# talmolab/VNL-Brax-Imitation

Measured on AMD Instinct MI355X. Metric: env-steps/sec (whole node), rodent imitation, num_envs=4096/GPU, higher is better.
Workload: dtype f32; 1 GPU; rodent imitation rollout, single groom clip, 4096 envs/GPU: intention-policy forward (HIP) -> RodentTracking.step (5 substeps, CG 6/6) -> auto-reset on -> Transition logging (unroll 20, the 20 steps replayed as one captured hipGraph); envs_per_gpu=4096, clips=1, parallelism=env-sharded x1, no data-path collective

## Files before the change

__graft_entry__.py:

```python
from __future__ import annotations

import os
import sys

ROOT = os.path.dirname(os.path.abspath(__file__))
if ROOT not in sys.path:
    sys.path.insert(0, ROOT)


def build() -> None:
    import vnl_brax_imitation_amd
    from vnl_brax_imitation_amd.csrc import build as hip_build

    from concurrent.futures import ThreadPoolExecutor

    with ThreadPoolExecutor(7) as pool:
        futs = {v: pool.submit(hip_build.build, variant=v)
                for v in ("product", "spill", "noblk", "nospec", "tail", "plain", "vmemplain")}
        paths = {v: f.result() for v, f in futs.items()}
    path = paths["product"]
    assert all(os.path.exists(p_) for p_ in paths.values()), paths
    from oracle import oracle as _oracle

    _oracle.build()
    from vnl_brax_imitation_amd import _lib

    _lib.load_library(path)
    print(f"[build] {path} ok; oracle ok")


def smoke() -> None:
    import numpy as np
    import torch

    sys.path.insert(0, os.path.join(ROOT, "tests"))
    import helpers as H
    from vnl_brax_imitation_amd.envs.rodent import RodentTracking

    assert torch.cuda.is_available(), "smoke() needs a HIP device"
    B = 256
    env = RodentTracking(H.reference_clip(), num_envs=B, device="cuda:0", **H.env_kwargs())
    rng = np.random.default_rng(0)
    sf = rng.integers(0, 235, B).astype(np.int32)
    noise = (1e-3 * rng.standard_normal((B, 74))).astype(np.float32)
    st = env.reset(start_frame=torch.from_numpy(sf), noise=torch.from_numpy(noise))
    act = np.clip(0.3 * rng.standard_normal((B, 30)), -1, 1).astype(np.float32)
    o = H.make_oracle(env, "f64")
    ost = o.env_reset(sf, noise)
    e_reset = H.scaled_err(st.pipeline_state.qacc_warmstart.cpu().numpy(), ost["qacc_warmstart"])
    e_obs = H.scaled_err(st.obs.cpu().numpy(), ost["obs"])
    import parity as P

    o32 = H.make_oracle(env, "f32")
    st, err, dev, rep, ost = P.control_step_follow(env, o, o32, sf, noise, act)
    torch.cuda.synchronize()
    print(f"[smoke] reset qacc err {e_reset:.2e}, obs err {e_obs:.2e}; control step vs oracle (following the product's "
          f"solver decisions): qvel err max {err['qvel'].max():.2e} median {np.median(err['qvel']):.2e}, qpos max "
          f"{err['qpos'].max():.2e}; reward {st.reward.mean().item():.5f} vs {ost['reward'].mean():.5f}")
    w = int(np.argmax(err["qvel"]))
    print(f"[smoke] worst env {w}: product vs float64 oracle {err['qvel'][w]:.2e}, float32 oracle vs float64 oracle "
          f"{dev['qvel'][w]:.2e} on the same env (bound: max(1e-5, {P.K_SENS} x that))")
    cp, co = P.compliance(err), P.compliance(dev)
    print(f"[smoke] envs within 1e-5 after ONE CONTROL STEP ({B} envs): product qpos {cp['qpos']:.3f} qvel {cp['qvel']:.3f} | "
          f"float32 oracle qpos {co['qpos']:.3f} qvel {co['qvel']:.3f}")
    env1 = RodentTracking(H.reference_clip(), num_envs=B, device="cuda:0", **{**H.env_kwargs(), "n_frames": 1})
    o1, o1_32 = H.make_oracle(env1, "f64"), H.make_oracle(env1, "f32")
    _, err1, dev1, rep1, _ = P.control_step_follow(env1, o1, o1_32, sf, noise, act)
    cp1, co1 = P.compliance(err1), P.compliance(dev1)
    print(f"[smoke] envs within 1e-5 after ONE SUBSTEP: product qpos {cp1['qpos']:.3f} qvel {cp1['qvel']:.3f} | float32 oracle "
          f"qpos {co1['qpos']:.3f} qvel {co1['qvel']:.3f}; followed decisions: {P.assert_legitimate(rep1)}")
    for f, idx in P.bound_violations(err1, dev1).items():
# ... 13 lines not shown
```

vnl-brax-imitation_amd/csrc/build.py:

```python
from __future__ import annotations

import os
import subprocess
import sys

HERE = os.path.dirname(os.path.abspath(__file__))
SOURCES = ["vnl_lib.hip", "vnl_policy.hip", "vnl_ppo.hip", "vnl_domain.hip"]
DEPS = SOURCES + ["vnl_env_kernels.h", "vnl_body.h", "vnl_types.h", "vnl_philox.h", "vnl_policy_train.h", "../../include/vnl.h"]
OUT = os.path.join(HERE, "libvnl.so")

VARIANTS = {
    "product": ("libvnl.so", ["-DVNL_KERNEL_ATTR=__attribute__((amdgpu_waves_per_eu(2,2)))"]),
    "prof": ("libvnl_prof.so", ["-DVNL_PROFILE", "-DVNL_KERNEL_ATTR=__attribute__((amdgpu_waves_per_eu(2,2)))"]),
    "knobs": ("libvnl_knobs.so", ["-DVNL_STAGE_KNOBS", "-DVNL_KERNEL_ATTR=__attribute__((amdgpu_waves_per_eu(2,2)))"]),
    "spill": ("libvnl_spill.so", ["-DVNL_KERNEL_ATTR=__attribute__((amdgpu_waves_per_eu(4,4)))"]),
    "noblk": ("libvnl_noblk.so", ["-DVNL_NO_BLK", "-DVNL_KERNEL_ATTR=__attribute__((amdgpu_waves_per_eu(2,2)))"]),
    "tail": ("libvnl_tail.so", ["-DVNL_SOLVER_TAIL", "-DVNL_KERNEL_ATTR=__attribute__((amdgpu_waves_per_eu(2,2)))"]),
    "plain": ("libvnl_plain.so", ["-DVNL_SOLVER_PLAIN", "-DVNL_KERNEL_ATTR=__attribute__((amdgpu_waves_per_eu(2,2)))"]),
    "vmemplain": ("libvnl_vmemplain.so", ["-DVNL_VMEM_PLAIN", "-DVNL_KERNEL_ATTR=__attribute__((amdgpu_waves_per_eu(2,2)))"]),
    "nospec": ("libvnl_nospec.so", ["-DVNL_NO_SPEC", "-DVNL_KERNEL_ATTR=__attribute__((amdgpu_waves_per_eu(2,2)))"]),
}
ENV_KERNELS = ("vnl_step_kernel", "vnl_reset_kernel", "vnl_reset_done_kernel")


def resource_usage(stderr_text: str) -> dict:
    out, name = {}, None
    for line in stderr_text.splitlines():
        if "Function Name:" in line:
            name = line.split("Function Name:")[1].split()[0]
            out[name] = {}
        elif name and "remark:" in line:
            body = line.split("remark:")[1].split("[-Rpass")[0].strip()
            key, _, val = body.rpartition(":")
            try:
                out[name][key.strip()] = int(val.strip())
            except ValueError:
                pass
    return out


def build(force: bool = False, verbose: bool = False, profile: bool = False, knobs: bool = False,
          variant: str | None = None) -> str:
    variant = variant or ("prof" if profile else ("knobs" if knobs else "product"))
    fname, defs = VARIANTS[variant]
    out = os.path.join(HERE, fname)
    deps = [os.path.join(HERE, d) for d in DEPS] + [os.path.abspath(__file__)]
    newest = max(os.path.getmtime(d) for d in deps)
    if not force and os.path.exists(out) and os.path.getmtime(out) >= newest:
        return out
    hipcc = os.environ.get("HIPCC", "/opt/rocm/bin/hipcc")
    objdir = os.path.join(HERE, "_obj", variant)
    os.makedirs(objdir, exist_ok=True)
    flags = ["-Rpass-analysis=kernel-resource-usage", "--offload-arch=gfx950", "-O3", "-fno-slp-vectorize", "-std=c++17", "-fPIC"] + \
        defs + os.environ.get("VNL_HIPCC_EXTRA", "").split()
    stamp = " ".join(flags)
    headers = [d for d in deps if not d.endswith(".hip")]
    SRC_DEPS = {"vnl_lib.hip": headers, "vnl_policy.hip": [h for h in headers if h.endswith("vnl.h")] + [os.path.join(HERE, "vnl_policy_train.h"), os.path.join(HERE, "vnl_philox.h")],
                "vnl_ppo.hip": [h for h in headers if h.endswith("vnl.h")] + [os.path.join(HERE, "vnl_policy_train.h")]}
    objs, remarks = [], ""
    for src in SOURCES:
        obj = os.path.join(objdir, src + ".o")
        rem = obj + ".remarks.txt"
        srcdeps = [os.path.join(HERE, src)] + [h for h in SRC_DEPS.get(src, headers) if os.path.exists(h)]
        fresh = (not force and os.path.exists(obj) and os.path.exists(rem) and
                 os.path.getmtime(obj) >= max(os.path.getmtime(d) for d in srcdeps) and
                 open(rem).readline().rstrip("\n") == stamp)
        if not fresh:
            cmd = [hipcc] + flags + ["-c", os.path.join(HERE, src), "-o", obj]
            if verbose:
                print(" ".join(cmd), file=sys.stderr)
            r = subprocess.run(cmd, stderr=subprocess.PIPE, text=True)
            if verbose or r.returncode:
# ... 48 lines not shown
```

vnl-brax-imitation_amd/csrc/vnl_body.h:

```cpp
#pragma once
#include <math.h>

#include "vnl_types.h"

#ifndef VNL_HD
#define VNL_HD __device__ __forceinline__
#endif
#include "vnl_philox.h"

#ifndef VNL_FORKJOIN_DEFINED
#define VNL_LANES 64
#define VNL_ROWS_PER_LANE 8
#define VNL_ROWS_SMALL 5
#define VNL_CHAIN_WIDTH 8
#define VNL_ROWSETS_1 1
#define VNL_ROWSETS_2 2
#define VNL_FOR(i, n) for (int i = (int)lane; i < (n); i += VNL_LANES)
#define VNL_SERIAL if (lane == 0)
#define VNL_SYNC() __builtin_amdgcn_fence(__ATOMIC_ACQ_REL, "wavefront")
#define VNL_SYNC_GLOBAL()                                     \
  do {                                                        \
    __builtin_amdgcn_fence(__ATOMIC_ACQ_REL, "wavefront");    \
    asm volatile("s_waitcnt vmcnt(0)" ::: "memory");          \
    __builtin_amdgcn_fence(__ATOMIC_ACQ_REL, "wavefront");    \
  } while (0)
#define VNL_LDS_DECL(name) extern __shared__ __align__(16) vreal name[]
VNL_HD float vnl_wave_sum(float x) {
#define VNL_DPP_STEP(ctrl) x += __builtin_bit_cast(float, __builtin_amdgcn_update_dpp(0, __builtin_bit_cast(int, x), ctrl, 0xf, 0xf, true))
  VNL_DPP_STEP(0xB1);
  VNL_DPP_STEP(0x4E);
  VNL_DPP_STEP(0x141);
  VNL_DPP_STEP(0x140);
#undef VNL_DPP_STEP
  x += __builtin_bit_cast(float, __builtin_amdgcn_update_dpp(0, __builtin_bit_cast(int, x), 0x142, 0xa, 0xf, false));
  x += __builtin_bit_cast(float, __builtin_amdgcn_update_dpp(0, __builtin_bit_cast(int, x), 0x143, 0xc, 0xf, false));
  return __builtin_bit_cast(float, __builtin_amdgcn_readlane(__builtin_bit_cast(int, x), 63));
}
VNL_HD float vnl_wave_sum16(float x) {
#define VNL_DPP_STEP(ctrl) x += __builtin_bit_cast(float, __builtin_amdgcn_update_dpp(0, __builtin_bit_cast(int, x), ctrl, 0xf, 0xf, true))
  VNL_DPP_STEP(0xB1);
  VNL_DPP_STEP(0x4E);
  VNL_DPP_STEP(0x141);
  VNL_DPP_STEP(0x140);
#undef VNL_DPP_STEP
  return __builtin_bit_cast(float, __builtin_amdgcn_readlane(__builtin_bit_cast(int, x), 0));
}
VNL_HD bool vnl_wave_any(bool x) { return __ballot(x) != 0ull; }
VNL_HD float vnl_wave_scan(float x) {
#define VNL_DPP_SCAN(ctrl, rmask) \
  x += __builtin_bit_cast(float, __builtin_amdgcn_update_dpp(0, __builtin_bit_cast(int, x), ctrl, rmask, 0xf, false))
  VNL_DPP_SCAN(0x111, 0xf);
  VNL_DPP_SCAN(0x112, 0xf);
  VNL_DPP_SCAN(0x114, 0xf);
  VNL_DPP_SCAN(0x118, 0xf);
// ... 84 lines not shown
}
VNL_HD V3 qrot(V3 v, Q4 q) {
  V3 u = v3(q.x, q.y, q.z);
  vreal uv = dot(u, v), uu = dot(u, u);
  V3 c = cross(u, v);
  return u * (vreal(2.) * uv) + v * (q.w * q.w - uu) + c * (vreal(2.) * q.w);
}
struct M3 {
  vreal a[9];
};
VNL_HD M3 qmat(Q4 q) {
  M3 m;
  vreal q00 = q.w * q.w, q01 = q.w * q.x, q02 = q.w * q.y, q03 = q.w * q.z;
  vreal q11 = q.x * q.x, q12 = q.x * q.y, q13 = q.x * q.z, q22 = q.y * q.y, q23 = q.y * q.z, q33 = q.z * q.z;
  m.a[0] = q00 + q11 - q22 - q33, m.a[1] = vreal(2.) * (q12 - q03), m.a[2] = vreal(2.) * (q13 + q02);
  m.a[3] = vreal(2.) * (q12 + q03), m.a[4] = q00 - q11 + q22 - q33, m.a[5] = vreal(2.) * (q23 - q01);
  m.a[6] = vreal(2.) * (q13 - q02), m.a[7] = vreal(2.) * (q23 + q01), m.a[8] = q00 - q11 - q22 + q33;
  return m;
}
VNL_HD V3 mmul(const M3& m, V3 v) {
  return V3{m.a[0] * v.x + m.a[1] * v.y + m.a[2] * v.z, m.a[3] * v.x + m.a[4] * v.y + m.a[5] * v.z,
            m.a[6] * v.x + m.a[7] * v.y + m.a[8] * v.z};
}
struct S6 {
  V3 a, l;
};
VNL_HD S6 operator+(S6 p, S6 q) { return S6{p.a + q.a, p.l + q.l}; }
VNL_HD S6 operator*(S6 p, vreal s) { return S6{p.a * s, p.l * s}; }
VNL_HD vreal dot(S6 p, S6 q) { return dot(p.a, q.a) + dot(p.l, q.l); }
VNL_HD S6 mcross(S6 u, S6 v) { return S6{cross(u.a, v.a), cross(u.l, v.a) + cross(u.a, v.l)}; }
VNL_HD S6 mcross_force(S6 v, S6 f) { return S6{cross(v.a, f.a) + cross(v.l, f.l), cross(v.a, f.l)}; }

#if defined(__HIP_DEVICE_COMPILE__)
#define VNL_CAS __attribute__((address_space(4)))
#define VNL_TO_CAS(T, p) ((const VNL_CAS T*)(unsigned long long)(p))
#define VNL_LAUNDER(p) asm volatile("" : "+s"(p))
#else
#define VNL_CAS
#define VNL_TO_CAS(T, p) ((const T*)(p))
#define VNL_LAUNDER(p)
#endif
#define MI(f) (SP::fixed ? SP::D.f : m.f)
#define LO(f) (SP::fixed ? SP::L.f : L.f)
#if defined(__HIP_DEVICE_COMPILE__)
#define VNL_GLOBAL_PTR(T, p) ((const __attribute__((address_space(1))) T*)(p))
#else
#define VNL_GLOBAL_PTR(T, p) ((const T*)(p))
#endif
#if defined(__HIP_DEVICE_COMPILE__) && !defined(VNL_VMEM_PLAIN)
#define VNL_PIN(x) asm volatile("" : "+v"(x))
#else
#define VNL_PIN(x) (void)(x)
#endif
#if defined(__HIP_DEVICE_COMPILE__) && !defined(VNL_SOLVER_PLAIN)
#define VNL_SOLVE_REGS 1
#else
#define VNL_SOLVE_REGS 0
#endif
#define VNL_BLK_REGS 2
#define VNL_LIMROW_REGS 2
#define VNL_SR_BLK 1
#define VNL_SR_LIMROW 2
struct VnlSolveRegs {
  int on;
  unsigned blk[2][VNL_BLK_REGS];
  int limrow[VNL_LIMROW_REGS];
};
template <class SP>
struct EnvWaveT {
  const VNL_CAS DevModel& m;
  const VNL_CAS DevEnv& ev;
  const DevState& st;
  const VNL_CAS WsLayout& L;
  vreal* s;
  unsigned e, lane;
  const VNL_CAS KernelConsts* kc;
  int* trace;
  VnlSolveRegs sr;
  VNL_HD EnvWaveT with_trace(int* t) const { return EnvWaveT{m, ev, st, L, s, e, lane, kc, t, sr}; }
  VNL_HD EnvWaveT fresh() const {
    const VNL_CAS KernelConsts* k = kc;
    VNL_LAUNDER(k);
    return EnvWaveT{k->m, k->ev, st, k->L, s, e, lane, k, trace, sr};
  }
  VNL_HD EnvWaveT with_solve_regs(bool with_limrow) const {
    EnvWaveT w = *this;
#if VNL_SOLVE_REGS
    const int cfg = MI(blk_cfg), tr = cfg & 15, tc = (cfg >> 4) & 15;
    const bool blk = blk_on();
#pragma unroll
    for (int t = 0; t < VNL_BLK_REGS; t++) {
      w.sr.blk[0][t] = (blk && t < tr) ? m.blk_tab[t * 64 + (int)lane] : 0u;
      w.sr.blk[1][t] = (blk && t < tc) ? m.blk_tab[(tr + t) * 64 + (int)lane] : 0u;
    }
#pragma unroll
    for (int q = 0; q < VNL_LIMROW_REGS; q++) {
      const int d = (int)lane + 64 * q;
      w.sr.limrow[q] = (with_limrow && d < MI(nv)) ? m.dof_limrow[d] : 0;
    }
#pragma unroll
    for (int t = 0; t < VNL_BLK_REGS; t++) asm volatile("" : "+v"(w.sr.blk[0][t]), "+v"(w.sr.blk[1][t]));
    if (with_limrow) {
#pragma unroll
      for (int q = 0; q < VNL_LIMROW_REGS; q++) asm volatile("" : "+v"(w.sr.limrow[q]));
    }
    w.sr.on = with_limrow ? (VNL_SR_BLK | VNL_SR_LIMROW) : VNL_SR_BLK;
// ... 654 lines not shown
        if (u < qd(q)) pb[u] = s + LDb + (u < d ? madr(anc_of(adr + u)) : 0);
#pragma unroll
      for (int t = 1; t < MAXD; t++) {
        if (t < qd(q) && vnl_wave_any(t <= d)) {
          vreal x[MAXD];
#pragma unroll
          for (int u = 1; u < t; u++) x[u] = pb[u][t - u];
          vreal acc = t <= d ? -s[own + t] : vreal(0.);
#pragma unroll
          for (int u = 1; u < t; u++) acc -= nn[u] * x[u];
          nn[t] = acc;
        }
      }
      VNL_SYNC();
#pragma unroll
      for (int t = 1; t < MAXD; t++)
        if (t < qd(q) && t <= d) s[own + t] = nn[t];
      VNL_SYNC();
    }
  }

  template <int NSET>
  VNL_HD void factor_aba(vreal h) const {
    constexpr int LW = 16;
    const int sc = (LO(Mgrad) + 3) & ~3;
    const int VS = vstore();
    vreal* g2 = fac2();
    const int nsteps = MI(fac_steps);
    v2r U[NSET][6], diag[NSET];
    vreal S[NSET][6];
    int dep[NSET], ftime[NSET], myline[NSET], adrs[NSET];
#ifdef VNL_VMEM_PLAIN
    const unsigned char* mt[NSET];
    unsigned nxt[NSET];
#else
    constexpr int NW = SP::fixed ? vnl_imax(vnl_fac_stride(SP::D.fac_steps) / 4, 1) : 4;
    const int nwords = vnl_fac_stride(nsteps) / 4;
    const auto* mw = VNL_GLOBAL_PTR(unsigned, m.fac_match);
    unsigned woff[NSET], win[NSET][NW], wcur[NSET];
    auto pick_word = [&](int q, int i) {
      unsigned r = win[q][0];
#pragma unroll
      for (int k = 1; k < NW; k++) {
        unsigned w = win[q][k];
        VNL_PIN(w);
        r = i == k ? w : r;
      }
      return r;
    };
    auto load_window = [&](int q, bool ok, int w0) {
#pragma unroll
      for (int i = 0; i < NW; i++) win[q][i] = (ok && w0 + i < nwords) ? mw[woff[q] + (unsigned)(w0 + i)] : 0u;
    };
    vreal inv2[NSET];
#endif
#pragma unroll
    for (int q = 0; q < NSET; q++) {
      const int a = (int)lane + q * VNL_LANES;
      const bool ok = a < MI(nv);
      const int aa = ok ? a : 0;
      const S6 c = ld6(LO(cdof) + 6 * aa), f = inert_mul(LO(P) + 10 * m.dof_body[aa], c);
      S[q][0] = c.a.x, S[q][1] = c.a.y, S[q][2] = c.a.z, S[q][3] = c.l.x, S[q][4] = c.l.y, S[q][5] = c.l.z;
      U[q][0] = v2r{f.a.x, f.a.x}, U[q][1] = v2r{f.a.y, f.a.y}, U[q][2] = v2r{f.a.z, f.a.z};
      U[q][3] = v2r{f.l.x, f.l.x}, U[q][4] = v2r{f.l.y, f.l.y}, U[q][5] = v2r{f.l.z, f.l.z};
      const vreal arm = par<P_ARM>(aa);
      diag[q] = v2r{arm, arm + h * par<P_DAMP>(aa)};
      adrs[q] = madr(aa), dep[q] = eadr(aa) - adrs[q];
      myline[q] = m.dof_fslot[aa];
      ftime[q] = ok ? m.dof_ftime[aa] : -1;
#ifdef VNL_VMEM_PLAIN
      mt[q] = m.fac_match + (size_t)aa * vnl_fac_stride(nsteps);
      nxt[q] = (ok && nsteps > 0) ? mt[q][0] : 0u;
#else
      woff[q] = (unsigned)(aa * nwords);
      load_window(q, ok, 0);
      wcur[q] = win[q][0];
      inv2[q] = vreal(0.);
#endif
    }
    VNL_SYNC();
    VNL_PROF(7);
    for (int step = 0; step < nsteps; step++) {
      unsigned cur[NSET];
#pragma unroll
      for (int q = 0; q < NSET; q++) {
#ifdef VNL_VMEM_PLAIN
        cur[q] = nxt[q];
        nxt[q] = (ftime[q] >= 0 && step + 1 < nsteps) ? mt[q][step + 1] : 0u;
#else
        cur[q] = wcur[q] & 0xffu, wcur[q] >>= 8;
#endif
        if (ftime[q] == step) {
          const int a = (int)lane + q * VNL_LANES;
          v2r D = diag[q];
#pragma unroll
          for (int i = 0; i < 6; i++) D += v2r{S[q][i], S[q][i]} * U[q][i];
          const v2r iv = v2r{vnl_recip(D[0]), vnl_recip(D[1])};
          vreal* ln = s + sc + myline[q] * LW;
          st4a(ln, U[q][0][0], U[q][0][1], U[q][1][0], U[q][1][1]);
          st4a(ln + 4, U[q][2][0], U[q][2][1], U[q][3][0], U[q][3][1]);
          st4a(ln + 8, U[q][4][0], U[q][4][1], U[q][5][0], U[q][5][1]);
          st4a(ln + 12, iv[0], iv[1], (vreal)(adrs[q] + dep[q]), vreal(0.));
          vreal* vs = s + VS + 12 * a;
          const v2r v0 = U[q][0] * iv, v1 = U[q][1] * iv, v2 = U[q][2] * iv, v3_ = U[q][3] * iv, v4 = U[q][4] * iv, v5 = U[q][5] * iv;
          st4a(vs, v0[0], v0[1], v1[0], v1[1]);
          st4a(vs + 4, v2[0], v2[1], v3_[0], v3_[1]);
          st4a(vs + 8, v4[0], v4[1], v5[0], v5[1]);
          s[LO(dinv) + a] = iv[0];
#ifdef VNL_VMEM_PLAIN
          g2[MI(nM) + a] = iv[1];
#else
          inv2[q] = iv[1];
#endif
        }
      }
      VNL_WAVE_FENCE();
      for (int pass = 0; pass < VNL_FAC_LINES; pass++) {
        bool more = false;
#pragma unroll
        for (int q = 0; q < NSET; q++) more = more || cur[q] != 0u;
        if (!vnl_wave_any(more)) break;
#pragma unroll
        for (int q = 0; q < NSET; q++) {
          if (cur[q] != 0u) {
            const int k = __builtin_ctz(cur[q]);
            cur[q] &= cur[q] - 1u;
            const vreal* ln = s + sc + k * LW;
            const R4 u0 = ld4a(ln), u1 = ld4a(ln + 4), u2 = ld4a(ln + 8), hd = ld4a(ln + 12);
            const v2r Uk[6] = {v2r{u0.x, u0.y}, v2r{u0.z, u0.w}, v2r{u1.x, u1.y}, v2r{u1.z, u1.w}, v2r{u2.x, u2.y}, v2r{u2.z, u2.w}};
            v2r pa = v2r{S[q][0], S[q][0]} * Uk[0], pb = v2r{S[q][1], S[q][1]} * Uk[1];
            pa += v2r{S[q][2], S[q][2]} * Uk[2], pb += v2r{S[q][3], S[q][3]} * Uk[3];
            pa += v2r{S[q][4], S[q][4]} * Uk[4], pb += v2r{S[q][5], S[q][5]} * Uk[5];
            const v2r Lk = (pa + pb) * v2r{hd.x, hd.y};
#pragma unroll
            for (int i = 0; i < 6; i++) U[q][i] -= Lk * Uk[i];
            s[LO(LD) + (int)hd.z - dep[q]] = Lk[0];
          }
        }
      }
      VNL_WAVE_FENCE();
#ifndef VNL_VMEM_PLAIN
      if ((step & 3) == 3) {
        const int wi = (step >> 2) + 1;
#pragma unroll
        for (int q = 0; q < NSET; q++) {
          if (!SP::fixed && wi % NW == 0) load_window(q, ftime[q] >= 0, wi);
          wcur[q] = pick_word(q, wi % NW);
        }
      }
#endif
    }
#ifndef VNL_VMEM_PLAIN
#pragma unroll
    for (int q = 0; q < NSET; q++)
      if (ftime[q] >= 0) g2[MI(nM) + (int)lane + q * VNL_LANES] = inv2[q];
#endif
    VNL_SYNC();
    VNL_PROF(8);
    VNL_PROF(9);
  }

  VNL_HD int vstore() const { return vnl_vstore(LO(P)); }
  VNL_HD int cvel_at() const { return vnl_cvel_at(LO(P), LO(smooth), MI(nbody), MI(nv)); }

  template <int NSET, bool GUESTS>
  VNL_HD void invert_aba(vreal* g2) const {
    const int VS = vstore();
    const unsigned char* an = (const unsigned char*)(s + LO(tab_anc));
    auto load_v = [&](int r, v2r* C) {
      const vreal* vs = s + VS + 12 * r;
      const R4 a = ld4a(vs), b = ld4a(vs + 4), c = ld4a(vs + 8);
      C[0] = v2r{a.x, a.y}, C[1] = v2r{a.z, a.w}, C[2] = v2r{b.x, b.y}, C[3] = v2r{b.z, b.w}, C[4] = v2r{c.x, c.y}, C[5] = v2r{c.z, c.w};
    };
#pragma unroll
    for (int q = 0; q < NSET; q++) {
      const int a = (int)lane + q * VNL_LANES;
      int row = a < MI(nv) ? a : -1, next = -1;
      if (GUESTS && q == 0 && m.fac_guest) next = m.fac_guest[lane];
      int adr = madr(row >= 0 ? row : 0), d = row >= 0 ? eadr(row) - adr : 0, tt = 0;
      v2r C[6];
      load_v(row >= 0 ? row : 0, C);
      int jn = an[adr + (d > 0 ? 1 : 0)];
      while (vnl_wave_any(row >= 0)) {
        if (row >= 0 && tt == d) {
          row = next, next = -1;
          if (row >= 0) {
            adr = madr(row), d = eadr(row) - adr, tt = 0;
            load_v(row, C);
            jn = an[adr + (d > 0 ? 1 : 0)];
          }
        }
        if (row >= 0 && tt < d) {
          const int j = jn;
          jn = an[adr + (tt + 2 <= d ? tt + 2 : d)];
          const S6 c = ld6(LO(cdof) + 6 * j);
          v2r V[6];
          load_v(j, V);
          v2r pa = v2r{c.a.x, c.a.x} * C[0], pb = v2r{c.a.y, c.a.y} * C[1];
          pa += v2r{c.a.z, c.a.z} * C[2], pb += v2r{c.l.x, c.l.x} * C[3];
          pa += v2r{c.l.y, c.l.y} * C[4], pb += v2r{c.l.z, c.l.z} * C[5];
          const v2r n = -(pa + pb);
#pragma unroll
          for (int i = 0; i < 6; i++) C[i] += n * V[i];
          tt++;
          s[LO(LD) + adr + tt] = n[0], g2[adr + tt] = n[1];
// ... 85 lines not shown
      vreal acc = s[in + a];
      const unsigned short* ea = (const unsigned short*)(s + LO(tab_madr)) + MI(nv);
      const vreal* ld = s + LDb - ST * da;
      int i = a + 1, iend = a + nd;
      constexpr int W = VNL_CHAIN_WIDTH;
      for (; i + W - 1 <= iend; i += W) {
        int e[W];
        vreal l[W], x[W];
#pragma unroll
        for (int u = 0; u < W; u++) e[u] = ea[i + u];
#pragma unroll
        for (int u = 0; u < W; u++) x[u] = s[in + i + u];
#pragma unroll
        for (int u = 0; u < W; u++) l[u] = ld[ST * e[u]];
        vreal p0 = vreal(0.), p1 = vreal(0.);
#pragma unroll
        for (int u = 0; u < W; u += 2) p0 += l[u] * x[u], p1 += l[u + 1] * x[u + 1];
        acc += p0 + p1;
      }
      if (i <= iend) {
        int e[W];
        vreal l[W], x[W];
#pragma unroll
        for (int u = 0; u < W; u++) {
          const int ii = i + u <= iend ? i + u : iend;
          e[u] = ea[ii], x[u] = s[in + ii];
        }
#pragma unroll
        for (int u = 0; u < W; u++) l[u] = ld[ST * e[u]];
        vreal p0 = vreal(0.), p1 = vreal(0.);
#pragma unroll
        for (int u = 0; u < W; u += 2) {
          p0 += i + u <= iend ? l[u] * x[u] : vreal(0.);
          p1 += i + u + 1 <= iend ? l[u + 1] * x[u + 1] : vreal(0.);
        }
        acc += p0 + p1;
      }
      s[out + a] = dmode == 1 ? acc * s[dinvb + ST * a] : (dmode == 2 ? acc / s[dinvb + ST * a] : acc);
    }
    VNL_SYNC();
  }

  template <int ST, bool COL>
  VNL_HD void blk_apply(int in, int out, int dmode, int LDb, int dinvb) const {
    const int cfg = MI(blk_cfg);
    const int trips = COL ? (cfg >> 4) & 15 : cfg & 15, steps = COL ? (cfg >> 12) & 15 : (cfg >> 8) & 15;
    const unsigned* tab = m.blk_tab + (COL ? (cfg & 15) * 64 : 0);
    constexpr int W = VNL_BLK_W, MAXT = 4;
#ifdef __HIP_DEVICE_COMPILE__
    unsigned pre[MAXT];
#pragma unroll
    for (int t = 0; t < MAXT; t++) pre[t] = t < trips ? tab[t * 64 + (int)lane] : 0u;
#endif
#pragma unroll
    for (int trip = 0; trip < MAXT; trip++) {
      if (trip >= trips) break;
      VNL_PERLANE(vreal, part);
      VNL_PERLANE(unsigned, dsc);
      VNL_FOR(l, VNL_WAVE_ITEMS(64)) {
#ifdef __HIP_DEVICE_COMPILE__
        const unsigned d = (VNL_SOLVE_REGS && (sr.on & VNL_SR_BLK) && trip < VNL_BLK_REGS) ? sr.blk[COL ? 1 : 0][trip] : pre[trip];
#else
        const unsigned d = tab[trip * 64 + l];
#endif
        const int n = (int)(d >> 16) & 15;
        vreal l_[W], x[W];
        if constexpr (!COL) {
          const int e0 = (int)(d & 0xffffu);
          const unsigned char* an = (const unsigned char*)(s + LO(tab_anc)) + e0;
          const vreal* row = s + LDb + ST * e0;
          int j[W];
#pragma unroll
          for (int u = 0; u < W; u++) j[u] = an[u], l_[u] = row[ST * u];
#pragma unroll
          for (int u = 0; u < W; u++) x[u] = s[in + j[u]];
        } else {
          const int i0 = (int)(d & 0x7fu), da = (int)(d >> 7) & 0x3f;
          const unsigned short* ea = (const unsigned short*)(s + LO(tab_madr)) + MI(nv) + i0;
          const vreal* ld = s + LDb - ST * da;
          int e[W];
#pragma unroll
          for (int u = 0; u < W; u++) e[u] = ea[u], x[u] = s[in + i0 + u];
#pragma unroll
          for (int u = 0; u < W; u++) l_[u] = ld[ST * e[u]];
        }
        vreal p0 = vreal(0.), p1 = vreal(0.);
#pragma unroll
        for (int u = 0; u < W; u++) {
          const vreal pr = u < n ? l_[u] * x[u] : vreal(0.);
          if (u & 1) p1 += pr;
          else p0 += pr;
        }
        VNL_AT(part, l) = p0 + p1;
        VNL_AT(dsc, l) = d;
      }
      VNL_SEG_SUM(part, dsc, steps);
      VNL_FOR(l, VNL_WAVE_ITEMS(64)) {
        const unsigned d = VNL_AT(dsc, l);
        if (d & (1u << 27)) {
          const int r = (int)(d >> 20) & 0x7f;
          const vreal acc = s[in + r] + VNL_AT(part, l);
          s[out + r] = dmode == 1 ? acc * s[dinvb + ST * r] : (dmode == 2 ? acc / s[dinvb + ST * r] : acc);
        }
      }
    }
    VNL_SYNC();
  }

  VNL_HD bool blk_on() const {
#ifdef VNL_NO_BLK
    return false;
#else
    return MI(blk_cfg) != 0;
#endif
  }
  VNL_HD void solve_inplace(int x, int LDb, int dinvb) const {
    if (blk_on()) {
      blk_apply<1, true>(x, LO(tmp2), 1, LDb, dinvb);
      blk_apply<1, false>(LO(tmp2), x, 0, LDb, dinvb);
      return;
    }
    col_apply(x, LO(tmp2), 1, LDb, dinvb);
    row_apply(LO(tmp2), x, false, LDb, dinvb);
  }
  VNL_HD void solve_inplace(int x) const { solve_inplace(x, LO(LD), LO(dinv)); }

  VNL_HD void mass_mul_factor(int vec, int out) const {
    if (blk_on()) {
      blk_apply<1, false>(vec, LO(tmp2), 2, LO(LD), LO(dinv));
      blk_apply<1, true>(LO(tmp2), out, 0, LO(LD), LO(dinv));
      return;
    }
    VNL_FOR(i, MI(nv)) {
      int adr = madr(i), dep = eadr(i) - adr;
      vreal acc = s[vec + i] + row_dot(adr, dep, vec, LO(LD));
      s[LO(tmp2) + i] = acc / s[LO(dinv) + i];
    }
    VNL_SYNC();
    col_apply(LO(tmp2), out, 0, LO(LD), LO(dinv));
  }

  VNL_HD void invert_both(vreal* g2) const {
    if (MI(nv) <= VNL_ROWSETS_1 * VNL_LANES) invert_aba<VNL_ROWSETS_1, false>(g2);
#if VNL_LANES == 64
    else if (m.fac_guest) invert_aba<VNL_ROWSETS_1, true>(g2);
#endif
    else invert_aba<VNL_ROWSETS_2, false>(g2);
  }

  VNL_HD int bias_forces() const {
    int nb6 = 6 * MI(nbody);
    int X0 = LO(P) + 10 * MI(nbody);
    dof_prefix(LO(qvel), LO(LD));
    const int cv = cvel_at();
    VNL_FOR(b, MI(nbody)) st6(cv + 6 * b, path_sum(LO(LD), m.body_pathseg + 8 * b));
    VNL_SYNC();
    VNL_PROF(2);
    int ca = X0;
// ... 544 lines not shown
      case VNL_ROUTE_ROWS36X2: factor_rows_at<VNL_ROWSETS_2, 36, 16, true>(true, Hb, dinvb, scb); break;
      default: factor_lds(Hb, dinvb, true);
    }
  }
  VNL_HD void newton_mass_mul(int v, int out) const {
    const int Mb = LO(newt_M);
    VNL_FOR(i, MI(nv)) {
      const int adr = madr(i), dep = eadr(i) - adr, nd = ndesc(i);
      vreal acc = s[Mb + adr] * s[v + i] + row_dot(adr, dep, v, Mb);
      for (int k = i + 1; k <= i + nd; k++) acc += s[Mb + eadr(k) - dep] * s[v + k];
      s[out + i] = acc;
    }
    VNL_SYNC();
  }

  VNL_HD void solve() const {
    const int nv = MI(nv), ne = MI(nefc);
    fresh().jac_mul(LO(qacc_smooth), LO(Jaref), true);
    vreal cost_s = fresh().constraint_cost(LO(Jaref));
    VNL_FOR(d, nv) s[LO(tmp) + d] = s[LO(qacc) + d] - s[LO(qacc_smooth) + d];
    VNL_SYNC();
    fresh().jac_mul(LO(tmp), LO(jv), false);
    for_live_rows([&](int r) { s[LO(jv) + r] += s[LO(Jaref) + r]; });
    vreal gw = vreal(0.);
    VNL_FOR(d, nv) gw += (s[LO(mv) + d] - s[LO(smooth) + d]) * s[LO(tmp) + d];
    gw = vnl_wave_sum(gw);
    VNL_SYNC();
    vreal cost_w = fresh().constraint_cost(LO(jv)) + vreal(0.5) * gw;
    bool use_warm = cost_w < cost_s;
    if (trace) {
      VNL_FOR(k, VNL_TRACE_ROWS) trace[k] = k == 0 ? (int)use_warm : 0;
    }
    VNL_FOR(d, nv) {
      s[LO(qacc) + d] = use_warm ? s[LO(qacc) + d] : s[LO(qacc_smooth) + d];
      s[LO(Ma) + d] = use_warm ? s[LO(mv) + d] : s[LO(smooth) + d];
    }
    if (use_warm) for_live_rows([&](int r) { s[LO(Jaref) + r] = s[LO(jv) + r]; });
    VNL_SYNC();
    VNL_PROF(14);
    vreal gauss = use_warm ? vreal(0.5) * gw : vreal(0.);
    vreal cost = fresh().constraint_force() + gauss;
    vreal prev_cost = INFINITY;
    vreal gg = vreal(0.), ss = vreal(0.), gp = vreal(0.);
    VNL_FOR(d, nv) {
      vreal g = s[LO(Ma) + d] - s[LO(smooth) + d] - s[LO(qfrc_c) + d];
      s[LO(grad) + d] = g, s[LO(Mgrad) + d] = g;
      gg += g * g;
    }
    gg = vnl_wave_sum(gg);
    VNL_SYNC();
    const bool newton = MI(solver_newton) != 0;
    if (newton) fresh().newton_solve(LO(Mgrad));
    else fresh().solve_inplace(LO(Mgrad));
    VNL_FOR(d, nv) {
      const vreal mg = s[LO(Mgrad) + d], gr = s[LO(grad) + d];
      s[LO(search) + d] = -mg;
      s[LO(mv) + d] = -gr;
      ss += mg * mg, gp += gr * mg;
    }
    ss = vnl_wave_sum(ss), gp = vnl_wave_sum(gp);
    VNL_SYNC();
    if (newton) fresh().newton_mass_mul(LO(search), LO(mv));
    VNL_PROF(15);

    for (int it = 0; it < MI(iterations); it++) {
      vreal improvement = (prev_cost - cost) / m.scale;
      vreal gradient = sqrt(gg) / m.scale;
      if (improvement < m.tolerance || gradient < m.tolerance) break;
      vreal smag = sqrt(ss) * m.scale;
      vreal gtol = m.tolerance * m.ls_tolerance * smag;
      VNL_PROF(16);
      fresh().jac_mul(LO(search), LO(jv), false);
      VNL_PROF(17);
      vreal qg1 = vreal(0.), qg2 = vreal(0.);
      VNL_FOR(d, nv) {
        vreal sd = s[LO(search) + d];
        qg1 += sd * s[LO(Ma) + d] - sd * s[LO(smooth) + d];
        qg2 += sd * s[LO(mv) + d];
      }
      qg1 = vnl_wave_sum(qg1), qg2 = vreal(0.5) * vnl_wave_sum(qg2);
      VNL_PROF(18);
      int* tr = (trace && it < VNL_TRACE_ITERS) ? trace + 8 + VNL_TRACE_REC * it : nullptr;
      if (trace) {
        VNL_SYNC();
        VNL_SERIAL { trace[1] = it + 1; }
      }
      const int nlive = num_live_rows();
      vreal alpha = (nlive <= (VNL_LANES < VNL_LIVE_MAX ? VNL_LANES : VNL_LIVE_MAX))
                        ? fresh().template line_search<1, true>(gauss, qg1, qg2, gtol, tr)
                        : (nlive <= (2 * VNL_LANES < VNL_LIVE_MAX ? 2 * VNL_LANES : VNL_LIVE_MAX))
                        ? fresh().template line_search<2, true>(gauss, qg1, qg2, gtol, tr)
                        : ((MI(nefc) <= 5 * VNL_LANES) ? fresh().template line_search<VNL_ROWS_SMALL>(gauss, qg1, qg2, gtol, tr)
                                                     : fresh().template line_search<VNL_ROWS_PER_LANE>(gauss, qg1, qg2, gtol, tr));
      VNL_FOR(d, nv) {
        s[LO(qacc) + d] += alpha * s[LO(search) + d];
        s[LO(Ma) + d] += alpha * s[LO(mv) + d];
      }
      VNL_PROF(19);
      for_live_rows([&](int r) { s[LO(Jaref) + r] += alpha * s[LO(jv) + r]; });
      VNL_SYNC();
      VNL_PROF(20);
#ifndef VNL_SOLVER_TAIL
      if (it + 1 >= MI(iterations) && !trace) {
        (void)fresh().constraint_force();
        VNL_PROF(22);
        break;
      }
#endif
      vreal g = vreal(0.);
      VNL_FOR(d, nv) g += (s[LO(Ma) + d] - s[LO(smooth) + d]) * (s[LO(qacc) + d] - s[LO(qacc_smooth) + d]);
      g = vnl_wave_sum(g);
      VNL_PROF(21);
      vreal ncost = fresh().constraint_force() + vreal(0.5) * g;
      VNL_PROF(22);
      prev_cost = cost, cost = ncost, gauss = vreal(0.5) * g;
      vreal d1 = vreal(0.);
      gg = vreal(0.);
      VNL_FOR(d, nv) {
        vreal gn = s[LO(Ma) + d] - s[LO(smooth) + d] - s[LO(qfrc_c) + d];
        d1 += gn * s[LO(Mgrad) + d];
        s[LO(grad) + d] = gn, s[LO(tmp) + d] = gn;
        gg += gn * gn;
      }
      d1 = vnl_wave_sum(d1), gg = vnl_wave_sum(gg);
      VNL_SYNC();
      VNL_PROF(23);
      if (newton) fresh().newton_solve(LO(tmp));
      else fresh().solve_inplace(LO(tmp));
      VNL_PROF(24);
      vreal d2 = vdot(LO(grad), LO(tmp));
      vreal beta = fmax(vreal(0.), (d2 - d1) / fmax(VNL_MINVAL, gp));
      if (newton) beta = vreal(0.);
      gp = d2;
      ss = vreal(0.);
      VNL_FOR(d, nv) {
        vreal mg = s[LO(tmp) + d];
        s[LO(Mgrad) + d] = mg;
        const vreal sn = -mg + beta * s[LO(search) + d];
        s[LO(search) + d] = sn;
        s[LO(mv) + d] = -s[LO(grad) + d] + beta * s[LO(mv) + d];
        ss += sn * sn;
      }
      ss = vnl_wave_sum(ss);
      VNL_SYNC();
      if (newton) fresh().newton_mass_mul(LO(search), LO(mv));
      VNL_PROF(25);
    }
  }

  VNL_HD void forward(const vreal* gwarm) const {
#ifdef VNL_VMEM_PLAIN
    const vreal* warm = gwarm ? gwarm : s + LO(qacc);
    VNL_FOR(d, MI(nv)) s[LO(tmp) + d] = warm[d];
    VNL_SYNC();
    VNL_FOR(d, MI(nv)) s[LO(qacc) + d] = s[LO(tmp) + d];
    VNL_SYNC();
#else
    if (gwarm) {
      const auto* gw = VNL_GLOBAL_PTR(vreal, gwarm);
      VNL_FOR(d, MI(nv)) s[LO(qacc) + d] = gw[d];
      VNL_SYNC();
    }
#endif
#ifdef VNL_STAGE_KNOBS
    for (int rep = 0; rep < m.dbg_count; rep++) {
      if (m.dbg_stage == 1) {
        kinematics();
        body_inertias(false);
        mass_matrix(vreal(0.));
        factor();
        invert_factor();
      } else if (m.dbg_stage == 2) {
        kinematics();
      } else if (m.dbg_stage == 3) {
        kinematics();
        body_inertias(false);
        mass_matrix(vreal(0.));
      } else if (m.dbg_stage == 4) {
        kinematics();
        body_inertias(false);
        mass_matrix(vreal(0.));
        factor();
      } else if (m.dbg_stage == 5) {
        kinematics();
        body_inertias(true);
        (void)bias_forces();
      } else if (m.dbg_stage == 14) {
        kinematics();
        body_inertias(false);
        mass_matrix(vreal(0.));
        factor(false);
      } else if (m.dbg_stage == 15) {
        kinematics();
        body_inertias(false);
        tree_accumulate(LO(P), 10);
        if (factor_pair_ok()) factor_both(m.dt);
// ... 485 lines not shown
```

Baseline: 2.589 million env-steps/s.

## Fuse solver dot products into update loops and batch LDS loads in factor/solve

```diff
diff --git a/__graft_entry__.py b/__graft_entry__.py
--- a/__graft_entry__.py
+++ b/__graft_entry__.py
@@ -14,9 +14,9 @@
 
     from concurrent.futures import ThreadPoolExecutor
 
-    with ThreadPoolExecutor(7) as pool:
+    with ThreadPoolExecutor(8) as pool:
         futs = {v: pool.submit(hip_build.build, variant=v)
-                for v in ("product", "spill", "noblk", "nospec", "tail", "plain", "vmemplain")}
+                for v in ("product", "spill", "noblk", "nospec", "tail", "plain", "vmemplain", "ldsplain")}
         paths = {v: f.result() for v, f in futs.items()}
     path = paths["product"]
     assert all(os.path.exists(p_) for p_ in paths.values()), paths
diff --git a/vnl-brax-imitation_amd/csrc/build.py b/vnl-brax-imitation_amd/csrc/build.py
--- a/vnl-brax-imitation_amd/csrc/build.py
+++ b/vnl-brax-imitation_amd/csrc/build.py
@@ -18,6 +18,7 @@
     "tail": ("libvnl_tail.so", ["-DVNL_SOLVER_TAIL", "-DVNL_KERNEL_ATTR=__attribute__((amdgpu_waves_per_eu(2,2)))"]),
     "plain": ("libvnl_plain.so", ["-DVNL_SOLVER_PLAIN", "-DVNL_KERNEL_ATTR=__attribute__((amdgpu_waves_per_eu(2,2)))"]),
     "vmemplain": ("libvnl_vmemplain.so", ["-DVNL_VMEM_PLAIN", "-DVNL_KERNEL_ATTR=__attribute__((amdgpu_waves_per_eu(2,2)))"]),
+    "ldsplain": ("libvnl_ldsplain.so", ["-DVNL_LDS_PLAIN", "-DVNL_KERNEL_ATTR=__attribute__((amdgpu_waves_per_eu(2,2)))"]),
     "nospec": ("libvnl_nospec.so", ["-DVNL_NO_SPEC", "-DVNL_KERNEL_ATTR=__attribute__((amdgpu_waves_per_eu(2,2)))"]),
 }
 ENV_KERNELS = ("vnl_step_kernel", "vnl_reset_kernel", "vnl_reset_done_kernel")
diff --git a/vnl-brax-imitation_amd/csrc/vnl_body.h b/vnl-brax-imitation_amd/csrc/vnl_body.h
--- a/vnl-brax-imitation_amd/csrc/vnl_body.h
+++ b/vnl-brax-imitation_amd/csrc/vnl_body.h
@@ -1,5 +1,8 @@
 #pragma once
 #include <math.h>
+#ifdef VNL_FORKJOIN_DEFINED
+#include <assert.h>
+#endif
 
 #include "vnl_types.h"
 
@@ -190,6 +193,11 @@
 #else
 #define VNL_PIN(x) (void)(x)
 #endif
+#if defined(__HIP_DEVICE_COMPILE__)
+#define VNL_OPAQUE(x) asm volatile("" : "+v"(x))
+#else
+#define VNL_OPAQUE(x) (void)(x)
+#endif
 #if defined(__HIP_DEVICE_COMPILE__) && !defined(VNL_SOLVER_PLAIN)
 #define VNL_SOLVE_REGS 1
 #else
@@ -950,7 +958,14 @@
 #pragma unroll
       for (int i = 0; i < NW; i++) win[q][i] = (ok && w0 + i < nwords) ? mw[woff[q] + (unsigned)(w0 + i)] : 0u;
     };
+#ifdef VNL_LDS_PLAIN
     vreal inv2[NSET];
+#endif
+#endif
+#ifndef VNL_LDS_PLAIN
+    v2r ivp[NSET];
+#pragma unroll
+    for (int q = 0; q < NSET; q++) ivp[q] = v2r{vreal(0.), vreal(0.)};
 #endif
 #pragma unroll
     for (int q = 0; q < NSET; q++) {
@@ -973,7 +988,9 @@
       woff[q] = (unsigned)(aa * nwords);
       load_window(q, ok, 0);
       wcur[q] = win[q][0];
+#ifdef VNL_LDS_PLAIN
       inv2[q] = vreal(0.);
+#endif
 #endif
     }
     VNL_SYNC();
@@ -989,7 +1006,6 @@
         cur[q] = wcur[q] & 0xffu, wcur[q] >>= 8;
 #endif
         if (ftime[q] == step) {
-          const int a = (int)lane + q * VNL_LANES;
           v2r D = diag[q];
 #pragma unroll
           for (int i = 0; i < 6; i++) D += v2r{S[q][i], S[q][i]} * U[q][i];
@@ -999,16 +1015,22 @@
           st4a(ln + 4, U[q][2][0], U[q][2][1], U[q][3][0], U[q][3][1]);
           st4a(ln + 8, U[q][4][0], U[q][4][1], U[q][5][0], U[q][5][1]);
           st4a(ln + 12, iv[0], iv[1], (vreal)(adrs[q] + dep[q]), vreal(0.));
+#ifndef VNL_LDS_PLAIN
+          ivp[q] = iv;
+#else
+          const int a = (int)lane + q * VNL_LANES;
           vreal* vs = s + VS + 12 * a;
           const v2r v0 = U[q][0] * iv, v1 = U[q][1] * iv, v2 = U[q][2] * iv, v3_ = U[q][3] * iv, v4 = U[q][4] * iv, v5 = U[q][5] * iv;
           st4a(vs, v0[0], v0[1], v1[0], v1[1]);
           st4a(vs + 4, v2[0], v2[1], v3_[0], v3_[1]);
           st4a(vs + 8, v4[0], v4[1], v5[0], v5[1]);
           s[LO(dinv) + a] = iv[0];
+#ifndef VNL_VMEM_PLAIN
+          inv2[q] = iv[1];
+#endif
+#endif
 #ifdef VNL_VMEM_PLAIN
-          g2[MI(nM) + a] = iv[1];
-#else
-          inv2[q] = iv[1];
+          g2[MI(nM) + (int)lane + q * VNL_LANES] = iv[1];
 #endif
         }
       }
@@ -1018,13 +1040,28 @@
 #pragma unroll
         for (int q = 0; q < NSET; q++) more = more || cur[q] != 0u;
         if (!vnl_wave_any(more)) break;
+#ifndef VNL_LDS_PLAIN
+        R4 lu0[NSET], lu1[NSET], lu2[NSET], lhd[NSET];
+#pragma unroll
+        for (int q = 0; q < NSET; q++) {
+          if (vnl_wave_any(cur[q] != 0u)) {
+            const vreal* ln = s + sc + (cur[q] != 0u ? __builtin_ctz(cur[q]) : 0) * LW;
+            lu0[q] = ld4a(ln), lu1[q] = ld4a(ln + 4), lu2[q] = ld4a(ln + 8), lhd[q] = ld4a(ln + 12);
+          }
+        }
+#endif
 #pragma unroll
         for (int q = 0; q < NSET; q++) {
           if (cur[q] != 0u) {
+#ifndef VNL_LDS_PLAIN
+            cur[q] &= cur[q] - 1u;
+            const R4 u0 = lu0[q], u1 = lu1[q], u2 = lu2[q], hd = lhd[q];
+#else
             const int k = __builtin_ctz(cur[q]);
             cur[q] &= cur[q] - 1u;
             const vreal* ln = s + sc + k * LW;
             const R4 u0 = ld4a(ln), u1 = ld4a(ln + 4), u2 = ld4a(ln + 8), hd = ld4a(ln + 12);
+#endif
             const v2r Uk[6] = {v2r{u0.x, u0.y}, v2r{u0.z, u0.w}, v2r{u1.x, u1.y}, v2r{u1.z, u1.w}, v2r{u2.x, u2.y}, v2r{u2.z, u2.w}};
             v2r pa = v2r{S[q][0], S[q][0]} * Uk[0], pb = v2r{S[q][1], S[q][1]} * Uk[1];
             pa += v2r{S[q][2], S[q][2]} * Uk[2], pb += v2r{S[q][3], S[q][3]} * Uk[3];
@@ -1048,7 +1085,24 @@
       }
 #endif
     }
+#ifndef VNL_LDS_PLAIN
+#pragma unroll
+    for (int q = 0; q < NSET; q++) {
+      if (ftime[q] >= 0) {
+        const int a = (int)lane + q * VNL_LANES;
+        const v2r iv = ivp[q];
+        vreal* vs = s + VS + 12 * a;
+        const v2r v0 = U[q][0] * iv, v1 = U[q][1] * iv, v2 = U[q][2] * iv, v3_ = U[q][3] * iv, v4 = U[q][4] * iv, v5 = U[q][5] * iv;
+        st4a(vs, v0[0], v0[1], v1[0], v1[1]);
+        st4a(vs + 4, v2[0], v2[1], v3_[0], v3_[1]);
+        st4a(vs + 8, v4[0], v4[1], v5[0], v5[1]);
+        s[LO(dinv) + a] = iv[0];
 #ifndef VNL_VMEM_PLAIN
+        g2[MI(nM) + a] = iv[1];
+#endif
+      }
+    }
+#elif !defined(VNL_VMEM_PLAIN)
 #pragma unroll
     for (int q = 0; q < NSET; q++)
       if (ftime[q] >= 0) g2[MI(nM) + (int)lane + q * VNL_LANES] = inv2[q];
@@ -1240,6 +1294,7 @@
 #pragma unroll
     for (int t = 0; t < MAXT; t++) pre[t] = t < trips ? tab[t * 64 + (int)lane] : 0u;
 #endif
+#ifdef VNL_LDS_PLAIN
 #pragma unroll
     for (int trip = 0; trip < MAXT; trip++) {
       if (trip >= trips) break;
@@ -1292,6 +1347,113 @@
         }
       }
     }
+#else
+    constexpr int PH = 2;
+#ifdef VNL_FORKJOIN_DEFINED
+    assert(in != out && (in + MI(nv) <= out || out + MI(nv) <= in));
+    assert(out + MI(nv) <= LDb || LDb + ST * MI(nM) <= out);
+    assert(out + MI(nv) <= dinvb || dinvb + ST * MI(nv) <= out);
+#endif
+#pragma unroll
+    for (int t0 = 0; t0 < MAXT; t0 += PH) {
+      if (t0 >= trips) break;
+      VNL_PERLANE(vreal, part[PH]);
+      VNL_PERLANE(unsigned, dsc[PH]);
+      VNL_PERLANE(vreal, xin[PH]);
+      VNL_PERLANE(vreal, dv[PH]);
+      VNL_FOR(l, VNL_WAVE_ITEMS(64)) {
+        unsigned d[PH];
+        int idx[PH][W];
+        vreal l_[PH][W], x[PH][W];
+#pragma unroll
+        for (int k = 0; k < PH; k++) {
+          const int trip = t0 + k;
+          if (trip >= trips) break;
+#ifdef __HIP_DEVICE_COMPILE__
+          d[k] = (VNL_SOLVE_REGS && (sr.on & VNL_SR_BLK) && trip < VNL_BLK_REGS) ? sr.blk[COL ? 1 : 0][trip] : pre[trip];
+#else
+          d[k] = tab[trip * 64 + l];
+#endif
+          if constexpr (!COL) {
+            const int e0 = (int)(d[k] & 0xffffu);
+            const unsigned char* an = (const unsigned char*)(s + LO(tab_anc)) + e0;
+            const vreal* row = s + LDb + ST * e0;
+#pragma unroll
+            for (int u = 0; u < W; u++) idx[k][u] = an[u], l_[k][u] = row[ST * u];
+          } else {
+            const int i0 = (int)(d[k] & 0x7fu);
+            const unsigned short* ea = (const unsigned short*)(s + LO(tab_madr)) + MI(nv) + i0;
+#pragma unroll
+            for (int u = 0; u < W; u++) idx[k][u] = ea[u], x[k][u] = s[in + i0 + u];
+          }
+          const int r = (int)(d[k] >> 20) & 0x7f;
+#ifdef VNL_FORKJOIN_DEFINED
+          assert(r < MI(nv));
+#endif
+          VNL_AT(xin[k], l) = s[in + r];
+          VNL_AT(dv[k], l) = dmode != 0 ? s[dinvb + ST * r] : vreal(0.);
+        }
+#pragma unroll
+        for (int k = 0; k < PH; k++) {
+          if (t0 + k >= trips) break;
+#pragma unroll
+          for (int u = 0; u < W; u++) VNL_PIN(idx[k][u]);
+        }
+#pragma unroll
+        for (int k = 0; k < PH; k++) {
+          if (t0 + k >= trips) break;
+          if constexpr (!COL) {
+#pragma unroll
+            for (int u = 0; u < W; u++) x[k][u] = s[in + idx[k][u]];
+          } else {
+            const vreal* ld = s + LDb - ST * ((int)(d[k] >> 7) & 0x3f);
+#pragma unroll
+            for (int u = 0; u < W; u++) l_[k][u] = ld[ST * idx[k][u]];
+          }
+        }
+#pragma unroll
+        for (int k = 0; k < PH; k++) {
+          if (t0 + k >= trips) break;
+#pragma unroll
+          for (int u = 0; u < W; u++) {
+            if constexpr (!COL) VNL_PIN(x[k][u]);
+            else VNL_PIN(l_[k][u]);
+          }
+        }
+#pragma unroll
+        for (int k = 0; k < PH; k++) {
+          if (t0 + k >= trips) break;
+          const int n = (int)(d[k] >> 16) & 15;
+          vreal p0 = vreal(0.), p1 = vreal(0.);
+#pragma unroll
+          for (int u = 0; u < W; u++) {
+            const vreal pr = u < n ? l_[k][u] * x[k][u] : vreal(0.);
+            if (u & 1) p1 += pr;
+            else p0 += pr;
+          }
+          VNL_AT(part[k], l) = p0 + p1;
+          VNL_AT(dsc[k], l) = d[k];
+        }
+      }
+#pragma unroll
+      for (int k = 0; k < PH; k++) {
+        if (t0 + k >= trips) break;
+        VNL_SEG_SUM(part[k], dsc[k], steps);
+      }
+      VNL_FOR(l, VNL_WAVE_ITEMS(64)) {
+#pragma unroll
+        for (int k = 0; k < PH; k++) {
+          if (t0 + k >= trips) break;
+          const unsigned d = VNL_AT(dsc[k], l);
+          if (d & (1u << 27)) {
+            const int r = (int)(d >> 20) & 0x7f;
+            const vreal acc = VNL_AT(xin[k], l) + VNL_AT(part[k], l);
+            s[out + r] = dmode == 1 ? acc * VNL_AT(dv[k], l) : (dmode == 2 ? acc / VNL_AT(dv[k], l) : acc);
+          }
+        }
+      }
+    }
+#endif
     VNL_SYNC();
   }
 
@@ -1942,13 +2104,27 @@
     const bool newton = MI(solver_newton) != 0;
     if (newton) fresh().newton_solve(LO(Mgrad));
     else fresh().solve_inplace(LO(Mgrad));
+#ifdef VNL_LDS_PLAIN
+    const bool qg_carried = false;
+#else
+    const bool qg_carried = !newton;
+#endif
+    vreal qg1c = vreal(0.), qg2c = vreal(0.);
     VNL_FOR(d, nv) {
       const vreal mg = s[LO(Mgrad) + d], gr = s[LO(grad) + d];
       s[LO(search) + d] = -mg;
       s[LO(mv) + d] = -gr;
       ss += mg * mg, gp += gr * mg;
+      if (qg_carried) {
+        vreal sd = -mg, md = -gr;
+        VNL_OPAQUE(sd);
+        VNL_OPAQUE(md);
+        qg1c += sd * s[LO(Ma) + d] - sd * s[LO(smooth) + d];
+        qg2c += sd * md;
+      }
     }
     ss = vnl_wave_sum(ss), gp = vnl_wave_sum(gp);
+    if (qg_carried) qg1c = vnl_wave_sum(qg1c), qg2c = vreal(0.5) * vnl_wave_sum(qg2c);
     VNL_SYNC();
     if (newton) fresh().newton_mass_mul(LO(search), LO(mv));
     VNL_PROF(15);
@@ -1962,13 +2138,16 @@
       VNL_PROF(16);
       fresh().jac_mul(LO(search), LO(jv), false);
       VNL_PROF(17);
-      vreal qg1 = vreal(0.), qg2 = vreal(0.);
-      VNL_FOR(d, nv) {
-        vreal sd = s[LO(search) + d];
-        qg1 += sd * s[LO(Ma) + d] - sd * s[LO(smooth) + d];
-        qg2 += sd * s[LO(mv) + d];
-      }
-      qg1 = vnl_wave_sum(qg1), qg2 = vreal(0.5) * vnl_wave_sum(qg2);
+      vreal qg1 = qg1c, qg2 = qg2c;
+      if (!qg_carried) {
+        qg1 = vreal(0.), qg2 = vreal(0.);
+        VNL_FOR(d, nv) {
+          vreal sd = s[LO(search) + d];
+          qg1 += sd * s[LO(Ma) + d] - sd * s[LO(smooth) + d];
+          qg2 += sd * s[LO(mv) + d];
+        }
+        qg1 = vnl_wave_sum(qg1), qg2 = vreal(0.5) * vnl_wave_sum(qg2);
+      }
       VNL_PROF(18);
       int* tr = (trace && it < VNL_TRACE_ITERS) ? trace + 8 + VNL_TRACE_REC * it : nullptr;
       if (trace) {
@@ -1982,10 +2161,23 @@
                         ? fresh().template line_search<2, true>(gauss, qg1, qg2, gtol, tr)
                         : ((MI(nefc) <= 5 * VNL_LANES) ? fresh().template line_search<VNL_ROWS_SMALL>(gauss, qg1, qg2, gtol, tr)
                                                      : fresh().template line_search<VNL_ROWS_PER_LANE>(gauss, qg1, qg2, gtol, tr));
+#ifdef VNL_LDS_PLAIN
       VNL_FOR(d, nv) {
         s[LO(qacc) + d] += alpha * s[LO(search) + d];
         s[LO(Ma) + d] += alpha * s[LO(mv) + d];
       }
+#else
+      vreal g = vreal(0.);
+      VNL_FOR(d, nv) {
+        vreal qa = s[LO(qacc) + d], ma = s[LO(Ma) + d];
+        qa += alpha * s[LO(search) + d];
+        ma += alpha * s[LO(mv) + d];
+        VNL_OPAQUE(qa);
+        VNL_OPAQUE(ma);
+        s[LO(qacc) + d] = qa, s[LO(Ma) + d] = ma;
+        g += (ma - s[LO(smooth) + d]) * (qa - s[LO(qacc_smooth) + d]);
+      }
+#endif
       VNL_PROF(19);
       for_live_rows([&](int r) { s[LO(Jaref) + r] += alpha * s[LO(jv) + r]; });
       VNL_SYNC();
@@ -1997,8 +2189,10 @@
         break;
       }
 #endif
+#ifdef VNL_LDS_PLAIN
       vreal g = vreal(0.);
       VNL_FOR(d, nv) g += (s[LO(Ma) + d] - s[LO(smooth) + d]) * (s[LO(qacc) + d] - s[LO(qacc_smooth) + d]);
+#endif
       g = vnl_wave_sum(g);
       VNL_PROF(21);
       vreal ncost = fresh().constraint_force() + vreal(0.5) * g;
@@ -2023,6 +2217,7 @@
       if (newton) beta = vreal(0.);
       gp = d2;
       ss = vreal(0.);
+#ifdef VNL_LDS_PLAIN
       VNL_FOR(d, nv) {
         vreal mg = s[LO(tmp) + d];
         s[LO(Mgrad) + d] = mg;
@@ -2031,7 +2226,26 @@
         s[LO(mv) + d] = -s[LO(grad) + d] + beta * s[LO(mv) + d];
         ss += sn * sn;
       }
+#else
+      qg1c = vreal(0.), qg2c = vreal(0.);
+      VNL_FOR(d, nv) {
+        vreal mg = s[LO(tmp) + d];
+        s[LO(Mgrad) + d] = mg;
+        vreal sn = -mg + beta * s[LO(search) + d];
+        vreal mn = -s[LO(grad) + d] + beta * s[LO(mv) + d];
+        VNL_OPAQUE(sn);
+        VNL_OPAQUE(mn);
+        s[LO(search) + d] = sn;
+        s[LO(mv) + d] = mn;
+        ss += sn * sn;
+        if (qg_carried) {
+          qg1c += sn * s[LO(Ma) + d] - sn * s[LO(smooth) + d];
+          qg2c += sn * mn;
+        }
+      }
+#endif
       ss = vnl_wave_sum(ss);
+      if (qg_carried) qg1c = vnl_wave_sum(qg1c), qg2c = vreal(0.5) * vnl_wave_sum(qg2c);
       VNL_SYNC();
       if (newton) fresh().newton_mass_mul(LO(search), LO(mv));
       VNL_PROF(25);
```

After: 2.672 million env-steps/s, median of 6. 1.03x the previous value.
